# szy4017/DeepSense6G_TII

Measured on NVIDIA B200. Metric: train samples/sec (fwd+bwd), higher is better.
Workload: dtype bf16

## Files before the change

### deepsense6g_tii_b200/_capi.py

```python
import ctypes
import os
from ctypes import POINTER, c_char_p, c_double, c_float, c_int32, c_int64, c_void_p

import torch

_HERE = os.path.dirname(os.path.abspath(__file__))
LIB_PATH = os.environ.get("DSF_LIB") or os.path.join(_HERE, "libdsfuse.so")

DSF_F32, DSF_BF16 = 0, 1
DSF_NCHW, DSF_NHWC = 0, 1
EPI_BIAS, EPI_RELU, EPI_RESIDUAL, EPI_ACCUM = 1, 2, 4, 8

SYMBOLS = [
    "dsf_version", "dsf_last_error", "dsf_launch_count", "dsf_check_device", "dsf_set_pdl", "dsf_set_sm_margin", "dsf_dropout_inplace", "dsf_tokens_fwd", "dsf_tokens_bwd",
    "dsf_layernorm_fwd", "dsf_layernorm_bwd", "dsf_gemm_bf16_nt", "dsf_gemm_bf16_tn", "dsf_gemm_set_impl", "dsf_gemm_f32",
    "dsf_colsum", "dsf_relu_bwd", "dsf_relu_bwd_colsum", "dsf_pack_block_weights", "dsf_softmax_fwd", "dsf_softmax_bwd", "dsf_attn_fwd", "dsf_attn_bwd", "dsf_attn_bwd_parts", "dsf_attn_set_impl", "dsf_attn_drop_words",
    "dsf_upsample_add_fwd", "dsf_upsample_add_bwd", "dsf_cast_f32_bf16", "dsf_opt_tiles", "dsf_adamw_ema_pack", "dsf_opt_upload_table", "dsf_chain_fwd", "dsf_chain_bwd",
    "dsf_stem_pack", "dsf_tail_fwd", "dsf_tail_bwd",
]


class Geom(ctypes.Structure):
    _fields_ = [(n, c_int32) for n in ("B", "S", "V", "A_h", "A_w", "C", "H", "W", "feat_dtype", "layout")]

# ... 31 lines not shown
                "(there is no CPU / PyTorch fallback for the fusion stage)" % LIB_PATH)
        L = ctypes.CDLL(LIB_PATH)
        L.dsf_last_error.restype = c_char_p
        L.dsf_version.restype = c_int32
        L.dsf_launch_count.restype = c_int64
        P = c_void_p
        sig = {
            "dsf_check_device": [],
            "dsf_tokens_fwd": [POINTER(Geom), P, P, P, P, P, P, P],
            "dsf_tokens_bwd": [POINTER(Geom), P, P, P, P, P, P, P, P, P, P],
            "dsf_layernorm_fwd": [P, P, P, P, c_int32, P, P, c_int32, c_int32, c_float, P],
            "dsf_layernorm_bwd": [P, c_int32, P, P, P, P, P, P, P, P, P, P, POINTER(Dropout), c_int32, c_int32, P],
            "dsf_dropout_inplace": [P, c_int64, POINTER(Dropout), P],
            "dsf_relu_bwd_colsum": [P, P, P, c_int32, c_int32, P],
            "dsf_pack_block_weights": [P] * 9 + [c_int32, c_int32] + [P] * 10,
            "dsf_gemm_bf16_nt": [P, c_int32, P, c_int32, P, c_int32, c_int32, P, P, c_int32, c_int32, c_int32, c_int32, POINTER(Dropout), P, P],
            "dsf_gemm_bf16_tn": [P, c_int32, P, c_int32, P, c_int32, c_int32, c_int32, c_int32, P, P],
            "dsf_gemm_f32": [POINTER(GemmF32Desc), P, P, P, P, P, P],
            "dsf_colsum": [P, c_int32, c_int32, P, c_int32, c_int32, P],
            "dsf_relu_bwd": [P, P, c_int32, c_int64, P],
            "dsf_softmax_fwd": [P, c_int64, c_int32, P],
            "dsf_softmax_bwd": [P, P, c_int64, c_int32, P],
            "dsf_attn_fwd": [P, P, P, c_int32, c_int32, c_int32, c_int32, POINTER(Dropout), P, P],
            "dsf_attn_bwd": [P, P, P, P, P, P, c_int32, c_int32, c_int32, c_int32, POINTER(Dropout), P, P],
            "dsf_attn_bwd_parts": [P, P, P, P, P, P, c_int32, c_int32, c_int32, c_int32, POINTER(Dropout), P, c_int32, P],
            "dsf_attn_set_impl": [c_int32],
            "dsf_set_pdl": [c_int32],
            "dsf_set_sm_margin": [c_int32],
            "dsf_gemm_set_impl": [c_int32],
            "dsf_upsample_add_fwd": [POINTER(Geom), P, P, P, P, P, P, P, P],
            "dsf_upsample_add_bwd": [POINTER(Geom), P, P, P, P, P, P],
# ... 83 lines not shown
def dropout_inplace(x, drop):
    _chk(lib().dsf_dropout_inplace(_p(x), x.numel(), _dp(drop), _stream()), "dsf_dropout_inplace")


def relu_bwd_colsum(dy, h, out):
    M, N = dy.shape
    _chk(lib().dsf_relu_bwd_colsum(_p(dy), _p(h), _p(out), M, N, _stream()), "dsf_relu_bwd_colsum")


def pack_block_weights(wq, wk, wv, wp, w1, w2, bq, bk, bv, outs):
    C, F = wq.shape[0], w1.shape[0]
    _chk(lib().dsf_pack_block_weights(_p(wq), _p(wk), _p(wv), _p(wp), _p(w1), _p(w2), _p(bq), _p(bk), _p(bv), C, F,
                                      *[_p(t) for t in outs], _stream()), "dsf_pack_block_weights")


def gemm_bf16_nt(A, B, C, bias=None, residual=None, relu=False, drop=None, relu_src=None):
    M, K = A.shape
    N = B.shape[0]
    flags = (EPI_BIAS if bias is not None else 0) | (EPI_RELU if relu else 0) | (EPI_RESIDUAL if residual is not None else 0)
    _chk(lib().dsf_gemm_bf16_nt(_p(A), A.stride(0), _p(B), B.stride(0), _p(C), C.stride(0), _dt(C), _p(bias), _p(residual),
                                M, N, K, flags, _dp(drop), _p(relu_src), _stream()), "dsf_gemm_bf16_nt")


def gemm_bf16_tn(A, B, C, colsum=None):
    M, Nout = A.shape
    Kout = B.shape[1]
    _chk(lib().dsf_gemm_bf16_tn(_p(A), A.stride(0), _p(B), B.stride(0), _p(C), C.stride(0), M, Nout, Kout, _p(colsum), _stream()),
         "dsf_gemm_bf16_tn")


def gemm_f32(desc, A, B, C, bias=None, residual=None):
    _chk(lib().dsf_gemm_f32(ctypes.byref(desc), _p(A), _p(B), _p(C), _p(bias), _p(residual), _stream()), "dsf_gemm_f32")


def colsum(X, out):
    M, N = X.shape
# ... 120 lines not shown
```

### deepsense6g_tii_b200/csrc/attn_api.cu

```cuda
#include <algorithm>
#include <atomic>

#include "tc_common.cuh"

namespace dsf {


__global__ void __launch_bounds__(256)
attn_delta_kernel(const __nv_bfloat16* __restrict__ y, const __nv_bfloat16* __restrict__ dy, float* __restrict__ delta, int B, int T,
                  int C, int nh) {
  pdl_trigger();
  pdl_wait();
  const int lane = threadIdx.x & 31;
  const int hs = C / nh, gl = hs / 8;
  const int nchunk = C / 8;
  for (int64_t row = (int64_t)blockIdx.x * 8 + (threadIdx.x >> 5); row < (int64_t)B * T; row += (int64_t)gridDim.x * 8) {
    const int b = (int)(row / T), t = (int)(row % T);
    for (int c0 = 0; c0 < nchunk; c0 += 32) {
      const int ch = c0 + lane;
      float acc = 0.f;
      if (ch < nchunk) {
        const uint4 a = __ldg(reinterpret_cast<const uint4*>(y + row * C + ch * 8));
        const uint4 d = __ldg(reinterpret_cast<const uint4*>(dy + row * C + ch * 8));
        const __nv_bfloat162* ap = reinterpret_cast<const __nv_bfloat162*>(&a);
        const __nv_bfloat162* dp = reinterpret_cast<const __nv_bfloat162*>(&d);
#pragma unroll
        for (int k = 0; k < 4; ++k) {
          const float2 af = __bfloat1622float2(ap[k]), df = __bfloat1622float2(dp[k]);
          acc += af.x * df.x + af.y * df.y;
        }
      }
      for (int o = gl >> 1; o > 0; o >>= 1) acc += __shfl_xor_sync(0xffffffffu, acc, o);
      if (ch < nchunk && (lane % gl) == 0) delta[((size_t)b * nh + (ch * 8) / hs) * T + t] = acc;
    }
  }
}

int attn_fwd_run(const void* qkv, void* y, float* lse, int B, int T, int C, int nh, const dsf_dropout* drop, uint32_t* bits, int force_nwg,
                 cudaStream_t st);
int attn_bwd_run(const void* qkv, const void* y, const void* dy, const float* lse, float* delta, void* dqkv, int B, int T, int C, int nh,
                 const dsf_dropout* drop, uint32_t* bits, int parts, cudaStream_t st);

int run_attn_delta(const void* y, const void* dy, float* delta, int B, int T, int C, int nh, cudaStream_t st) {
  launch_pdl(attn_delta_kernel, dim3(std::min(cdiv(B * T, 8), num_sms() * 8)), dim3(256), 0, st, (const __nv_bfloat16*)y, (const __nv_bfloat16*)dy,
             delta, B, T, C, nh);
// ... 70 lines not shown
```

### deepsense6g_tii_b200/csrc/common.cuh

```cuda
#pragma once
#include <cuda_bf16.h>
#include <cuda_runtime.h>
#include <stdint.h>
#include <stdio.h>

#include "../../include/dsfuse.h"

namespace dsf {

void set_error(const char* fmt, ...);
int check_launch(const char* what);

#define DSF_REQUIRE(cond, ...)              \
  do {                                      \
    if (!(cond)) {                          \
      ::dsf::set_error(__VA_ARGS__);        \
      return DSF_EINVAL;                    \
    }                                       \
  } while (0)

inline bool aligned16(const void* p) { return (reinterpret_cast<uintptr_t>(p) & 15u) == 0; }
inline int cdiv(int a, int b) { return (a + b - 1) / b; }
inline int64_t cdiv64(int64_t a, int64_t b) { return (a + b - 1) / b; }

// ... 118 lines not shown
  }
}
__device__ __forceinline__ void drop_scale4(const DropArgs& a, uint64_t e4, float (&m)[4]) {
  float m8[8];
  drop_scale8(a, e4 >> 1, m8);
  const int h = (int)(e4 & 1) * 4;
#pragma unroll
  for (int k = 0; k < 4; ++k) m[k] = m8[h + k];
}

__device__ __forceinline__ uint32_t pack_bf16x2(float lo, float hi) {
  __nv_bfloat162 t = __floats2bfloat162_rn(lo, hi);
  return *reinterpret_cast<uint32_t*>(&t);
}

}
```

### deepsense6g_tii_b200/csrc/gemm_api.cu

```cuda
#include <algorithm>
#include <atomic>

#include "tc_common.cuh"

namespace dsf {

typedef CUresult (*PFN_encodeTiled)(CUtensorMap*, CUtensorMapDataType, cuuint32_t, void*, const cuuint64_t*, const cuuint64_t*,
                                    const cuuint32_t*, const cuuint32_t*, CUtensorMapInterleave, CUtensorMapSwizzle,
                                    CUtensorMapL2promotion, CUtensorMapFloatOOBfill);

static PFN_encodeTiled get_encode() {
  static PFN_encodeTiled fn = nullptr;
  if (!fn) {
    void* p = nullptr;
    cudaDriverEntryPointQueryResult q;
    if (cudaGetDriverEntryPoint("cuTensorMapEncodeTiled", &p, cudaEnableDefault, &q) == cudaSuccess && q == cudaDriverEntryPointSuccess)
      fn = (PFN_encodeTiled)p;
  }
  return fn;
}

int make_tmap_bf16(CUtensorMap* m, const void* base, int rows, int cols, int ld, int box_rows) {
  PFN_encodeTiled enc = get_encode();
  if (!enc) { set_error("cuTensorMapEncodeTiled entry point not available"); return DSF_ELAUNCH; }
// ... 14 lines not shown
  cuuint64_t gdim[2] = {(cuuint64_t)cols, (cuuint64_t)rows};
  cuuint64_t gstr[1] = {(cuuint64_t)ld * es};
  cuuint32_t box[2] = {(cuuint32_t)box_cols, (cuuint32_t)box_rows};
  cuuint32_t estr[2] = {1u, 1u};
  CUresult r = enc(m, dtype == DSF_F32 ? CU_TENSOR_MAP_DATA_TYPE_FLOAT32 : CU_TENSOR_MAP_DATA_TYPE_BFLOAT16, 2, const_cast<void*>(base), gdim,
                   gstr, box, estr, CU_TENSOR_MAP_INTERLEAVE_NONE, CU_TENSOR_MAP_SWIZZLE_128B, CU_TENSOR_MAP_L2_PROMOTION_L2_256B,
                   CU_TENSOR_MAP_FLOAT_OOB_FILL_NONE);
  if (r != CUDA_SUCCESS) { set_error("cuTensorMapEncodeTiled(2d) failed (%d) rows=%d cols=%d ld=%d box=%dx%d", (int)r, rows, cols, ld, box_cols, box_rows); return DSF_ELAUNCH; }
  return DSF_OK;
}

}

namespace dsf {
int gemm_nt_run(const void* A, int lda, const void* B, int ldb, void* C, int ldc, int c_dtype, const float* bias, const float* residual, int M,
                int N, int K, int flags, const dsf_dropout* drop, const void* relu_src, bool pairs, cudaStream_t st);
int gemm_tn_run(const void* A, int lda, const void* B, int ldb, float* C, int ldc, int M, int Nout, int Kout, float* colsum, cudaStream_t st);
static std::atomic<int> g_gemm_impl{0};
}

using namespace dsf;

extern "C" int dsf_gemm_set_impl(int32_t impl) {
  DSF_REQUIRE(impl == 0 || impl == 2, "gemm_set_impl: impl must be 0 (default: CTA pairs where the shape allows) or 2 (single-CTA tiles only)");
  g_gemm_impl.store(impl, std::memory_order_relaxed);
  return DSF_OK;
}

extern "C" int dsf_gemm_bf16_nt(const void* A, int32_t lda, const void* B, int32_t ldb, void* C, int32_t ldc, int32_t c_dtype,
                                const float* bias, const float* residual, int32_t M, int32_t N, int32_t K, int32_t epi_flags,
                                const dsf_dropout* drop, const void* relu_src, void* stream) {
  DSF_REQUIRE(A && B && C, "gemm_bf16_nt: NULL pointer");
  DSF_REQUIRE(M > 0 && N > 0 && K > 0, "gemm_bf16_nt: non-positive extent");
  DSF_REQUIRE(K % 64 == 0, "gemm_bf16_nt: K=%d must be a multiple of 64", K);
  DSF_REQUIRE(N % 64 == 0, "gemm_bf16_nt: N=%d must be a multiple of 64", N);
  DSF_REQUIRE(lda % 8 == 0 && ldb % 8 == 0 && ldc % 8 == 0 && lda >= K && ldb >= K && ldc >= N, "gemm_bf16_nt: bad leading dimensions");
  DSF_REQUIRE(aligned16(A) && aligned16(B) && aligned16(C) && aligned16(bias) && aligned16(residual), "gemm_bf16_nt: 16-byte alignment required");
  DSF_REQUIRE(c_dtype == DSF_F32 || c_dtype == DSF_BF16, "gemm_bf16_nt: bad c_dtype %d", c_dtype);
  DSF_REQUIRE(!(epi_flags & DSF_EPI_BIAS) || bias, "gemm_bf16_nt: bias flag without bias pointer");
  DSF_REQUIRE(!(epi_flags & DSF_EPI_RESIDUAL) || residual, "gemm_bf16_nt: residual flag without residual pointer");
  DSF_REQUIRE(!(epi_flags & DSF_EPI_ACCUM), "gemm_bf16_nt: ACCUM is not supported on the NT path");
  DSF_REQUIRE(!drop || (drop->p >= 0.f && drop->p < 1.f), "gemm_bf16_nt: dropout p must be in [0, 1)");
  DSF_REQUIRE(!relu_src || aligned16(relu_src), "gemm_bf16_nt: relu_src must be 16-byte aligned");
  return gemm_nt_run(A, lda, B, ldb, C, ldc, c_dtype, bias, residual, M, N, K, epi_flags, drop, relu_src,
                     g_gemm_impl.load(std::memory_order_relaxed) == 0, (cudaStream_t)stream);
}

extern "C" int dsf_gemm_bf16_tn(const void* A, int32_t lda, const void* B, int32_t ldb, float* C, int32_t ldc, int32_t M,
                                int32_t Nout, int32_t Kout, float* colsum_a, void* stream) {
  DSF_REQUIRE(A && B && C, "gemm_bf16_tn: NULL pointer");
  DSF_REQUIRE(M > 0 && Nout > 0 && Kout > 0, "gemm_bf16_tn: non-positive extent");
  DSF_REQUIRE(Nout % 64 == 0 && Kout % 64 == 0, "gemm_bf16_tn: output extents (%d, %d) must be multiples of 64", Nout, Kout);
  DSF_REQUIRE(lda % 8 == 0 && ldb % 8 == 0 && lda >= Nout && ldb >= Kout && ldc >= Kout, "gemm_bf16_tn: bad leading dimensions");
  DSF_REQUIRE(aligned16(A) && aligned16(B) && aligned16(C), "gemm_bf16_tn: 16-byte alignment required");
  return gemm_tn_run(A, lda, B, ldb, C, ldc, M, Nout, Kout, colsum_a, (cudaStream_t)stream);
}
```

### deepsense6g_tii_b200/csrc/gemm_tc2.cu

```cuda
#include <algorithm>
#include <cstdlib>

#include "tc_common.cuh"

namespace dsf {

using namespace tc;

int make_tmap_bf16(CUtensorMap* m, const void* base, int rows, int cols, int ld, int box_rows);
int make_tmap_2d(CUtensorMap* m, const void* base, int dtype, int rows, int cols, int ld, int box_cols, int box_rows);

constexpr int G2_BM = 128, G2_BK = 64, G2_THREADS = 320;

struct EpiArgs2 {
  void* C;
  int ldc;
  int c_dtype;
  const float* bias;
  const float* residual;
  int flags;
  int N;
  const __nv_bfloat16* relu_src;
  int ablate;
  DropArgs drop;
};

__device__ __forceinline__ void epi_store32(const EpiArgs2& e, int row, int n, const uint32_t (&r)[32]) {
  float v[32];
#pragma unroll
  for (int j = 0; j < 32; ++j) v[j] = __uint_as_float(r[j]);
  if (e.flags & DSF_EPI_BIAS) {
#pragma unroll
    for (int j = 0; j < 32; j += 4) {
      const float4 b = __ldg(reinterpret_cast<const float4*>(e.bias + n + j));
      v[j] += b.x; v[j + 1] += b.y; v[j + 2] += b.z; v[j + 3] += b.w;
    }
  }
  if (e.flags & DSF_EPI_RELU) {
#pragma unroll
// ... 53 lines not shown
#pragma unroll
    for (int j = 0; j < 32; j += 8) {
      float m[8];
      drop_scale8(e.drop, e8 + (j >> 3), m);
#pragma unroll
      for (int k = 0; k < 8; ++k) v[j + k] *= m[k];
    }
  }
  if ((e.flags & DSF_EPI_RESIDUAL) && row_ok) {
    const float4* rp = reinterpret_cast<const float4*>(e.residual + (size_t)row * e.ldc + n);
#pragma unroll
    for (int j = 0; j < 8; ++j) {
      const float4 t = rp[j];
      v[4 * j] += t.x; v[4 * j + 1] += t.y; v[4 * j + 2] += t.z; v[4 * j + 3] += t.w;
    }
  }
}

template <int BN, int STAGES, bool STAGED = true>
struct G2Smem {
  static constexpr int A_BYTES = G2_BM * G2_BK * 2;
  static constexpr int B_BYTES = BN * G2_BK * 2;
  static constexpr int STAGE_BYTES = A_BYTES + B_BYTES;
  static constexpr int STAGING_OFF = STAGES * STAGE_BYTES;
  static constexpr int STAGING_BYTES = STAGED ? 8 * 2 * 4096 : 0;
  static constexpr int BAR_OFF = STAGING_OFF + STAGING_BYTES;
  static constexpr int DYN = BAR_OFF + (2 * STAGES + 4) * 8 + 16 + 1024;
  static constexpr uint32_t TMEM_COLS = 2 * BN < 32 ? 32 : 2 * BN;
  static_assert(DYN <= 232448, "shared memory budget");
};
// ... 63 lines not shown
          if (elect_one()) {
#pragma unroll
            for (int k = 0; k < G2_BK / 16; ++k) tc_mma_bf16(acc, da + (uint32_t)(k * 2), db + (uint32_t)(k * 2), idesc, k == 0 ? first : 1u);
            tc_commit(bar_empty + s * 8);
          }
          __syncwarp();
        }
        if (elect_one()) tc_commit(acc_full + ab * 8);
        __syncwarp();
      }
    }
  } else {
    const int q = warp & 3;
    const int ch = (warp - 2) >> 2;
    epi.drop = resolve_drop(epi.drop);
    constexpr int NSPLIT = BN >= 128 ? 2 : 1;
    constexpr int HALF = BN / NSPLIT;
    int i = 0, nbox = 0;
    for (int tile = blockIdx.x; tile < total; tile += gridDim.x, ++i) {
      const int ab = i & 1;
      const int m0 = (tile % m_tiles) * G2_BM, n0 = (tile / m_tiles) * BN;
      mbar_wait(acc_full + ab * 8, (i >> 1) & 1);
      tc_fence_after();
      if (ch >= NSPLIT || m0 + q * 32 >= M || (epi.ablate & 1)) {
        tc_fence_before();
        __syncwarp();
        if (lane == 0) mbar_arrive(acc_empty + ab * 8);
        continue;
      }
      const int row = m0 + q * 32 + lane;
      const uint32_t tacc = tmem_base + ab * BN + ((uint32_t)(q * 32) << 16) + ch * HALF;
      const uint32_t stg = base + L::STAGING_OFF + (warp - 2) * 8192;
      const int CW = epi.c_dtype == DSF_F32 ? 32 : 64;
#pragma unroll 1
      for (int c = 0; c < HALF; c += CW, ++nbox) {
        const uint32_t sbuf = stg + (nbox & 1) * 4096;
        if (lane == 0) bulk_wait_read<1>();
        __syncwarp();
        const int ncol = n0 + ch * HALF + c;
        uint32_t w[32];
        if (epi.c_dtype == DSF_F32) {
          uint32_t r[32];
          tmem_ld32(tacc + c, r);
          tmem_wait_ld();
          float v[32];
          epi_math32(epi, row, ncol, r, v, row < M);
#pragma unroll
          for (int j = 0; j < 32; ++j) w[j] = __float_as_uint(v[j]);
        } else {
#pragma unroll
          for (int hh = 0; hh < 2; ++hh) {
            uint32_t r[32];
            tmem_ld32(tacc + c + hh * 32, r);
            tmem_wait_ld();
            float v[32];
            epi_math32(epi, row, ncol + hh * 32, r, v, row < M);
#pragma unroll
            for (int j = 0; j < 16; ++j) w[hh * 16 + j] = pack_bf16x2(v[2 * j], v[2 * j + 1]);
          }
        }
        if (!(epi.ablate & 8)) {
#pragma unroll
        for (int j = 0; j < 8; ++j) {
          const uint32_t dst = sbuf + lane * 128 + ((j ^ (lane & 7)) << 4);
          asm volatile("st.shared.v4.b32 [%0], {%1, %2, %3, %4};" ::"r"(dst), "r"(w[4 * j]), "r"(w[4 * j + 1]), "r"(w[4 * j + 2]), "r"(w[4 * j + 3])
                       : "memory");
        }
        fence_proxy_async();
        } else {
          uint32_t acc = 0;
#pragma unroll
          for (int j = 0; j < 32; ++j) acc ^= w[j];
          if (acc == 0x12345678u) asm volatile("st.shared.b32 [%0], %1;" ::"r"(sbuf), "r"(acc) : "memory");
        }
// ... 185 lines not shown
            for (int k = 0; k < G2_BK / 16; ++k) tc_mma_bf16_pair(acc, da + (uint32_t)(k * 2), db + (uint32_t)(k * 2), idesc, k == 0 ? first : 1u);
            tc_commit_pair(bar_empty + s * 8);
          }
          __syncwarp();
        }
        if (elect_one()) tc_commit_pair(acc_full + ab * 8);
        __syncwarp();
      }
    }
  } else {
    const int q = warp & 3;
    const int ch = (warp - 2) >> 2;
    epi.drop = resolve_drop(epi.drop);
    constexpr int HALF = BN / 2;
    const uint32_t acc_empty0 = mapa_u32(acc_empty, 0);
    int i = 0, nbox = 0;
    const uint32_t rbuf = base + L::RES_OFF + (warp - 2) * 4096, rbar = base + L::RBAR_OFF + (warp - 2) * 8;
    int nres = 0;
    bool r_inflight = false;
    auto chunks_of = [&](int uu, int& cm0, int& cn0, int& clo, int& chi) -> bool {
      int t2, a0, a1, p2, off2, w2;
      unit_of(uu, t2, a0, a1, p2);
      if (n_split > 1) nsub_of(uu, t2, off2, w2);
      else { off2 = 0; w2 = BN; }
      cm0 = (t2 % m_tiles) * 256 + (int)rank * G2_BM;
      cn0 = (t2 / m_tiles) * BN + off2;
      const int hu = w2 / 2;
      clo = hu >= 32 ? ch * hu : 0;
      chi = hu >= 32 ? clo + hu : (ch == 0 ? w2 : 0);
      return p2 == 0 && cm0 + q * 32 < M && !(epi.ablate & 1) && clo < chi;
// ... 6 lines not shown
      }
      r_inflight = true;
    };
    if (RTMA && pair < total) {
      int cm0, cn0, clo, chi;
      if (chunks_of(pair, cm0, cn0, clo, chi)) issue_res(cn0 + clo, cm0 + q * 32);
    }
    for (int u = pair; u < total; u += n_pairs, ++i) {
      int tile, kb0, kb1, part;
      unit_of(u, tile, kb0, kb1, part);
      int n_off, width;
      if (n_split > 1) nsub_of(u, tile, n_off, width);
      else { n_off = 0; width = BN; }
      const int ab = i & 1;
      const int m0 = (tile % m_tiles) * 256 + (int)rank * G2_BM, n0 = (tile / m_tiles) * BN + n_off;
      mbar_wait(acc_full + ab * 8, (i >> 1) & 1);
      tc_fence_after();
      if (part != 0) {
        const int row = m0 + q * 32 + lane;
        const uint32_t tacc = tmem_base + ab * BN + ((uint32_t)(q * 32) << 16) + ch * HALF;
        EpiArgs2 e2 = epi;
        if (part == 2) e2.flags &= ~(DSF_EPI_BIAS | DSF_EPI_RESIDUAL);
        if (m0 + q * 32 < M) {
#pragma unroll 1
          for (int c = 0; c < HALF; c += 32) {
            uint32_t r[32];
            tmem_ld32(tacc + c, r);
            tmem_wait_ld();
            float v[32];
            const int ncol = n0 + ch * HALF + c;
            epi_math32(e2, row, ncol, r, v, row < M);
            if (row < M) {
              float* cp = reinterpret_cast<float*>(epi.C) + (size_t)row * epi.ldc + ncol;
#pragma unroll
              for (int j = 0; j < 32; j += 4) red_add_v4(cp + j, v[j], v[j + 1], v[j + 2], v[j + 3]);
            }
          }
        }
      } else
      if (m0 + q * 32 < M && !(epi.ablate & 1)) {
        const int row = m0 + q * 32 + lane;
        const uint32_t tacc = tmem_base + ab * BN + ((uint32_t)(q * 32) << 16);
        const uint32_t stg = base + L::STAGING_OFF + (warp - 2) * 8192;
        const int CW = epi.c_dtype == DSF_F32 ? 32 : 64;
        const int half_u = width / 2;
        const int c_lo = half_u >= CW ? ch * half_u : 0;
        const int c_hi = half_u >= CW ? c_lo + half_u : (ch == 0 ? width : 0);
#pragma unroll 1
        for (int c = c_lo; c < c_hi; c += CW, ++nbox) {
          const uint32_t sbuf = stg + (nbox & 1) * 4096;
          if (lane == 0) bulk_wait_read<1>();
          __syncwarp();
          const int ncol = n0 + c;
          uint32_t w[32];
          if (RTMA) {
            if (!r_inflight) issue_res(ncol, m0 + q * 32);
            mbar_wait(rbar, nres & 1);
            ++nres;
            float rr[32];
#pragma unroll
            for (int j = 0; j < 8; ++j) {
              const uint32_t src = rbuf + lane * 128 + ((j ^ (lane & 7)) << 4);
// ... 13 lines not shown
            float v[32];
            EpiArgs2 e2 = epi;
            e2.flags &= ~DSF_EPI_RESIDUAL;
            epi_math32(e2, row, ncol, r, v, row < M);
#pragma unroll
            for (int j = 0; j < 32; ++j) w[j] = __float_as_uint(v[j] + rr[j]);
          } else if (epi.c_dtype == DSF_F32) {
            uint32_t r[32];
            tmem_ld32(tacc + c, r);
            tmem_wait_ld();
            float v[32];
            epi_math32(epi, row, ncol, r, v, row < M);
#pragma unroll
            for (int j = 0; j < 32; ++j) w[j] = __float_as_uint(v[j]);
          } else {
#pragma unroll
            for (int hh = 0; hh < 2; ++hh) {
              uint32_t r[32];
              tmem_ld32(tacc + c + hh * 32, r);
              tmem_wait_ld();
              float v[32];
              epi_math32(epi, row, ncol + hh * 32, r, v, row < M);
#pragma unroll
              for (int j = 0; j < 16; ++j) w[hh * 16 + j] = pack_bf16x2(v[2 * j], v[2 * j + 1]);
            }
          }
#pragma unroll
          for (int j = 0; j < 8; ++j) {
            const uint32_t dst = sbuf + lane * 128 + ((j ^ (lane & 7)) << 4);
            asm volatile("st.shared.v4.b32 [%0], {%1, %2, %3, %4};" ::"r"(dst), "r"(w[4 * j]), "r"(w[4 * j + 1]), "r"(w[4 * j + 2]), "r"(w[4 * j + 3])
                         : "memory");
          }
          fence_proxy_async();
          __syncwarp();
          if (lane == 0) {
            tma_store_2d(&tmC, sbuf, ncol, m0 + q * 32);
            bulk_commit();
          }
        }
      }
      tc_fence_before();
      __syncwarp();
      if (lane == 0) mbar_arrive_cluster(acc_empty0 + ab * 8);
    }
    if (lane == 0) bulk_wait<0>();
  }
  tc_fence_before();
  cluster_sync_all();
  if (warp == 1) tmem_dealloc_pair(tmem_base, L::TMEM_COLS);
}



template <int BN, int STAGES>
struct TnSmem : G2Smem<BN, STAGES, false> {
// ... 150 lines not shown
  const int tiles = cdiv(Nout, G2_BM) * cdiv(Kout, BN);
  int splits = std::max(1, std::min(cdiv(M, 2 * G2_BK), num_sms() / std::max(1, tiles)));
  int m_chunk = cdiv(cdiv(M, splits), G2_BK) * G2_BK;
  splits = cdiv(M, m_chunk);
  dim3 grid(cdiv(Kout, BN), cdiv(Nout, G2_BM), splits);
  launch_pdl(gemm_tn2_kernel<BN, STAGES>, grid, dim3(G2_THREADS), L::DYN, st, tmA, tmB, C, ldc, M, Nout, Kout, m_chunk, colsum);
  return check_launch("gemm_tn2");
}

static const bool g_nt_tail_nsplit = getenv("DSF_GEMM_TAIL_NSPLIT") ? atoi(getenv("DSF_GEMM_TAIL_NSPLIT")) != 0 : true;

static const bool g_nt_res_tma = getenv("DSF_GEMM_RES_TMA") ? atoi(getenv("DSF_GEMM_RES_TMA")) != 0 : true;

template <int BN, int STAGES, bool RTMA = false>
static int launch_nt3(const CUtensorMap& tmA, const CUtensorMap& tmB, const CUtensorMap& tmC, const EpiArgs2& epi, int M, int N, int K,
                      cudaStream_t st, const void* Bptr = nullptr, int ldb = 0) {
  using L = G3Smem<BN, STAGES, RTMA>;
  static bool configured_on[64] = {};
  bool& configured = per_device_flag(configured_on);
  if (!configured) {
    if (cudaFuncSetAttribute(gemm_nt3_kernel<BN, STAGES, RTMA>, cudaFuncAttributeMaxDynamicSharedMemorySize, L::DYN) != cudaSuccess)
      return check_launch("gemm_nt3/attr");
    configured = true;
  }
  CUtensorMap tmR = tmC;
  if (RTMA) {
    if (int e = make_tmap_2d(&tmR, epi.residual, DSF_F32, M, N, epi.ldc, 32, 32)) return e;
  }
  const int m_tiles = cdiv(M, 256), n_tiles = N / BN;
  const int tiles = m_tiles * n_tiles;
  const int pairs = std::min(tiles, num_sms() / 2);
  int tail_start = tiles;
  const int tail_split = 1;
  const int rem = tiles % pairs;
  int n_split = 1;
  CUtensorMap tmBt = tmB;
  if (g_nt_tail_nsplit && tail_split == 1 && BN == 256 && Bptr != nullptr && rem > 0 && tiles > pairs) {
    for (int ns = 4; ns >= 2; ns >>= 1) {
      if (rem * ns <= pairs) { n_split = ns; break; }
    }
    if (n_split > 1) {
      tail_start = tiles - rem;
      if (int e = make_tmap_bf16(&tmBt, Bptr, N, K, ldb, BN / n_split / 2)) return e;
    }
  }
  launch_pdl(gemm_nt3_kernel<BN, STAGES, RTMA>, dim3(2 * pairs), dim3(G2_THREADS), L::DYN, st, tmA, tmB, tmC, tmBt, tmR, epi, M, N, K, m_tiles,
             n_tiles, tail_start, tail_split, n_split);
  return check_launch("gemm_nt3");
}

static int pick_bn_nt(int M, int N) {
  const int sms = num_sms();
  const int m_tiles = cdiv(M, G2_BM);
  int best = 64;
  double best_cost = 1e30;
  const int cands[3] = {256, 128, 64};
  const double tile_eff[3] = {1.0, 0.85, 0.6};
  for (int i = 0; i < 3; ++i) {
    const int bn = cands[i];
    if (N % bn) continue;
    const int tiles = m_tiles * (N / bn);
    const double cost = (double)cdiv(tiles, sms) * bn / tile_eff[i];
    if (cost < best_cost) { best_cost = cost; best = bn; }
  }
  return best;
}

int gemm_nt_run(const void* A, int lda, const void* B, int ldb, void* C, int ldc, int c_dtype, const float* bias, const float* residual, int M,
                int N, int K, int flags, const dsf_dropout* drop, const void* relu_src, bool pairs, cudaStream_t st) {
  static const int ablate = [] {
    const int v = getenv("DSF_GEMM_ABLATE") ? atoi(getenv("DSF_GEMM_ABLATE")) : 0;
    if (v) fprintf(stderr, "dsfuse: DSF_GEMM_ABLATE=%d is set: tensor-core GEMM results are INVALID (timing diagnostics only)\n", v);
    return v;
  }();
  CUtensorMap tmA, tmB;
  if (pairs && N % 128 == 0 && M > 128) {
    const int BN3 = (N % 256 == 0) ? 256 : 128;
    if (int e = make_tmap_bf16(&tmA, A, M, K, lda, G2_BM)) return e;
    if (int e = make_tmap_bf16(&tmB, B, N, K, ldb, BN3 / 2)) return e;
    CUtensorMap tmC3;
    if (int e = make_tmap_2d(&tmC3, C, c_dtype, M, N, ldc, c_dtype == DSF_F32 ? 32 : 64, 32)) return e;
    EpiArgs2 epi3{C, ldc, c_dtype, bias, residual, flags, N, reinterpret_cast<const __nv_bfloat16*>(relu_src), ablate, make_drop(drop)};
    if (BN3 == 256 && g_nt_res_tma && c_dtype == DSF_F32 && (flags & DSF_EPI_RESIDUAL) && residual != nullptr && !ablate)
      return launch_nt3<256, 4, true>(tmA, tmB, tmC3, epi3, M, N, K, st, B, ldb);
    if (BN3 == 256) return launch_nt3<256, 5>(tmA, tmB, tmC3, epi3, M, N, K, st, B, ldb);
    if (g_nt_res_tma && c_dtype == DSF_F32 && (flags & DSF_EPI_RESIDUAL) && residual != nullptr && !ablate)
      return launch_nt3<128, 5, true>(tmA, tmB, tmC3, epi3, M, N, K, st);
    return launch_nt3<128, 6>(tmA, tmB, tmC3, epi3, M, N, K, st);
  }
  const int BN = pick_bn_nt(M, N);
  if (int e = make_tmap_bf16(&tmA, A, M, K, lda, G2_BM)) return e;
  if (int e = make_tmap_bf16(&tmB, B, N, K, ldb, BN)) return e;
  CUtensorMap tmC;
  if (int e = make_tmap_2d(&tmC, C, c_dtype, M, N, ldc, c_dtype == DSF_F32 ? 32 : 64, 32)) return e;
  EpiArgs2 epi{C, ldc, c_dtype, bias, residual, flags, N, reinterpret_cast<const __nv_bfloat16*>(relu_src), ablate, make_drop(drop)};
  if (BN == 256) return launch_nt2<256, 3>(tmA, tmB, tmC, epi, M, N, K, st);
  if (BN == 128) return launch_nt2<128, 4>(tmA, tmB, tmC, epi, M, N, K, st);
  return launch_nt2<64, 5>(tmA, tmB, tmC, epi, M, N, K, st);
}

int gemm_tn_run(const void* A, int lda, const void* B, int ldb, float* C, int ldc, int M, int Nout, int Kout, float* colsum, cudaStream_t st) {
  const int BN = (Kout % 256 == 0) ? 256 : ((Kout % 128 == 0) ? 128 : 64);
  CUtensorMap tmA, tmB;
  if (int e = make_tmap_bf16(&tmA, A, M, Nout, lda, G2_BK)) return e;
  if (int e = make_tmap_bf16(&tmB, B, M, Kout, ldb, G2_BK)) return e;
  if (BN == 256) return launch_tn2<256, 4>(tmA, tmB, C, ldc, M, Nout, Kout, colsum, st);
  if (BN == 128) return launch_tn2<128, 6>(tmA, tmB, C, ldc, M, Nout, Kout, colsum, st);
  return launch_tn2<64, 8>(tmA, tmB, C, ldc, M, Nout, Kout, colsum, st);
}

// ... 2 lines not shown
```

### deepsense6g_tii_b200/functional.py

```python
import math
import os

import torch
from torch.autograd.function import once_differentiable

from . import _capi as K
from ._capi import EPI_ACCUM, EPI_BIAS, EPI_RELU, EPI_RESIDUAL, GemmF32Desc

PER_BLOCK = ("ln1.weight", "ln1.bias", "ln2.weight", "ln2.bias",
             "attn.key.weight", "attn.key.bias", "attn.query.weight", "attn.query.bias",
             "attn.value.weight", "attn.value.bias", "attn.proj.weight", "attn.proj.bias",
             "mlp.0.weight", "mlp.0.bias", "mlp.2.weight", "mlp.2.bias")


def param_names(n_layer):
    names = ["pos_emb"]
    for i in range(n_layer):
        names += ["blocks.%d.%s" % (i, n) for n in PER_BLOCK]
    return names + ["ln_f.weight", "ln_f.bias"]


def _f32_linear_desc(M, N, Kd, flags, trans=None):
    return GemmF32Desc(M, N, Kd, 1, 1, 0, 0, Kd, 1, 0, 0, Kd, 1, 0, 0, N, 1, 1.0, flags)

# ... 358 lines not shown
            dwqkv, dwp, dw1, dw2, dbqkv, dbp, db1, db2, dg1, dbt1, dg2, dbt2 = block_views(i)
            dwqkv, dwp, dw1, dw2 = dwqkv.view(3 * C, C), dwp.view(C, C), dw1.view(F, C), dw2.view(C, F)
            fork(lambda: K.gemm_bf16_tn(dxa, st.a, dw2))
            da = torch.empty(M, F, device=dev, dtype=bf)
            K.gemm_bf16_nt(dxa, st.w2_t, da, relu_src=st.a)

            fork(lambda: K.gemm_bf16_tn(da, st.h2, dw1, colsum=db1))
            dh2 = torch.empty(M, C, device=dev, dtype=dh_dt)
            K.gemm_bf16_nt(da, st.w1_t, dh2)
            dx_mid = torch.empty(M, C, device=dev, dtype=f32)
            dxm = torch.empty(M, C, device=dev, dtype=bf)
            K.layernorm_bwd(dh2, st.x_mid, ln2w, st.mean2, st.rstd2, dx, dx_mid, dg2, dbt2, dx_bf16=dxm, dx_colsum=dbp,
                            byprod_drop=self._drop("proj", i))
            fork(lambda: K.gemm_bf16_tn(dxm, st.y, dwp))
            dy = torch.empty(M, C, device=dev, dtype=bf)
            K.gemm_bf16_nt(dxm, st.wp_t, dy)
            dqkv = torch.empty(M, 3 * C, device=dev, dtype=bf)
            delta = torch.empty(self.B, self.nh, self.T, device=dev, dtype=f32)
            if side is None:
                K.attn_bwd(st.qkv, st.y, dy, st.lse, delta, dqkv, self.B, self.T, C, self.nh, self._drop("attn", i), st.drop_bits)
            else:
                adrop = self._drop("attn", i)
                K.attn_bwd(st.qkv, st.y, dy, st.lse, delta, dqkv, self.B, self.T, C, self.nh, adrop, st.drop_bits, parts=1)
                fork(lambda: K.attn_bwd(st.qkv, st.y, dy, st.lse, delta, dqkv, self.B, self.T, C, self.nh, adrop, st.drop_bits, parts=4), side_q)
                K.attn_bwd(st.qkv, st.y, dy, st.lse, delta, dqkv, self.B, self.T, C, self.nh, adrop, st.drop_bits, parts=2)
                join(side_q)

            fork(lambda: K.gemm_bf16_tn(dqkv, st.h1, dwqkv, colsum=dbqkv))
            dh1 = torch.empty(M, C, device=dev, dtype=dh_dt)
            K.gemm_bf16_nt(dqkv, st.wqkv_t, dh1)
            join_pending()
            if side is not None:
                ev_blk = torch.cuda.Event()
                ev_blk.record(side)
                pending = (ev_blk, i, (st, da, dxm, dqkv))
            dx = torch.empty(M, C, device=dev, dtype=f32)
            prev = block_views(i - 1) if i > 0 else None
            K.layernorm_bwd(dh1, st.x_in, ln1w, st.mean1, st.rstd1, dx_mid, dx, dg1, dbt1,
# ... 387 lines not shown
```

### include/dsfuse.h

```cpp
#ifndef DSFUSE_H_
#define DSFUSE_H_

#include <stdint.h>

#ifdef __cplusplus
extern "C" {
#endif

#define DSF_VERSION 100

enum { DSF_F32 = 0, DSF_BF16 = 1 };
enum { DSF_NCHW = 0, DSF_NHWC = 1 };
enum {
  DSF_OK = 0,
  DSF_EINVAL = 1,
  DSF_ELAUNCH = 2,
  DSF_EARCH = 3,
  DSF_EUNSUPPORTED = 4
};

enum {
  DSF_EPI_BIAS = 1,
  DSF_EPI_RELU = 2,
  DSF_EPI_RESIDUAL = 4,
// ... 33 lines not shown

int dsf_tokens_bwd(const dsf_geom* g, const float* dx, const void* dres_img, const void* dres_lidar,
                   const void* dres_radar, void* dimg, void* dlidar, void* dradar, float* dgps,
                   float* dpos_emb, void* stream);

int dsf_layernorm_fwd(const float* x, const float* gamma, const float* beta, void* y, int32_t y_dtype,
                      float* mean, float* rstd, int32_t M, int32_t C, float eps, void* stream);
int dsf_layernorm_bwd(const void* dy, int32_t dy_dtype, const float* x, const float* gamma,
                      const float* mean, const float* rstd, const float* dx_add, float* dx_out,
                      float* dgamma, float* dbeta, void* dx_bf16, float* dx_colsum,
                      const dsf_dropout* byprod_drop, int32_t M, int32_t C, void* stream);

int dsf_gemm_bf16_nt(const void* A, int32_t lda, const void* B, int32_t ldb, void* C, int32_t ldc,
                     int32_t c_dtype, const float* bias, const float* residual, int32_t M, int32_t N,
                     int32_t K, int32_t epi_flags, const dsf_dropout* drop, const void* relu_src,
                     void* stream);
int dsf_gemm_bf16_tn(const void* A, int32_t lda, const void* B, int32_t ldb, float* C, int32_t ldc,
                     int32_t M, int32_t Nout, int32_t Kout, float* colsum_a, void* stream);
int dsf_gemm_set_impl(int32_t impl);

typedef struct {
  int32_t M, N, K;
  int32_t nb1, nb2;
  int64_t a_b1, a_b2, a_m, a_k;
  int64_t b_b1, b_b2, b_n, b_k;
  int64_t c_b1, c_b2, c_m, c_n;
  float alpha;
  int32_t epi_flags;
} dsf_gemm_f32_desc;
int dsf_gemm_f32(const dsf_gemm_f32_desc* d, const float* A, const float* B, float* C,
                 const float* bias, const float* residual, void* stream);
// ... 80 lines not shown
```

Baseline: 1321.

## Fuse attention-backward delta row-dot into the dy GEMM epilogue

The GEMM that produces dy = dxm·Wp^T now also computes the per-head row dot product of dy with y in its epilogue and writes delta directly. This removes the separate delta pass that re-read y and dy (attn_bwd parts 1/6 now skip it). The epilogue gains extra y loads and reductions, and the tile width choices are constrained so each tile covers whole head groups, which may lower GEMM efficiency.

```diff
diff --git a/deepsense6g_tii_b200/_capi.py b/deepsense6g_tii_b200/_capi.py
--- a/deepsense6g_tii_b200/_capi.py
+++ b/deepsense6g_tii_b200/_capi.py
@@ -69,7 +69,8 @@
             "dsf_dropout_inplace": [P, c_int64, POINTER(Dropout), P],
             "dsf_relu_bwd_colsum": [P, P, P, c_int32, c_int32, P],
             "dsf_pack_block_weights": [P] * 9 + [c_int32, c_int32] + [P] * 10,
-            "dsf_gemm_bf16_nt": [P, c_int32, P, c_int32, P, c_int32, c_int32, P, P, c_int32, c_int32, c_int32, c_int32, POINTER(Dropout), P, P],
+            "dsf_gemm_bf16_nt": [P, c_int32, P, c_int32, P, c_int32, c_int32, P, P, c_int32, c_int32, c_int32, c_int32, POINTER(Dropout), P,
+                                 P, P, c_int32, c_int32, P],
             "dsf_gemm_bf16_tn": [P, c_int32, P, c_int32, P, c_int32, c_int32, c_int32, c_int32, P, P],
             "dsf_gemm_f32": [POINTER(GemmF32Desc), P, P, P, P, P, P],
             "dsf_colsum": [P, c_int32, c_int32, P, c_int32, c_int32, P],
@@ -183,12 +184,20 @@
                                       *[_p(t) for t in outs], _stream()), "dsf_pack_block_weights")
 
 
-def gemm_bf16_nt(A, B, C, bias=None, residual=None, relu=False, drop=None, relu_src=None):
+def gemm_bf16_nt(A, B, C, bias=None, residual=None, relu=False, drop=None, relu_src=None, dot_src=None, dot_out=None):
     M, K = A.shape
     N = B.shape[0]
     flags = (EPI_BIAS if bias is not None else 0) | (EPI_RELU if relu else 0) | (EPI_RESIDUAL if residual is not None else 0)
+    dot_T = dot_nh = 0
+    if dot_out is not None:
+        _req(dot_out, torch.float32, "dot_out")
+        if (dot_out.dim() != 3 or dot_out.shape[0] * dot_out.shape[2] != M or dot_src is None or dot_src.dtype != torch.bfloat16
+                or dot_src.shape != C.shape or dot_src.stride() != C.stride()):
+            raise RuntimeError("gemm_bf16_nt: dot_out must be (B, nh, T) with B*T = M rows and dot_src bf16 with C's shape and strides")
+        dot_nh, dot_T = dot_out.shape[1], dot_out.shape[2]
     _chk(lib().dsf_gemm_bf16_nt(_p(A), A.stride(0), _p(B), B.stride(0), _p(C), C.stride(0), _dt(C), _p(bias), _p(residual),
-                                M, N, K, flags, _dp(drop), _p(relu_src), _stream()), "dsf_gemm_bf16_nt")
+                                M, N, K, flags, _dp(drop), _p(relu_src), _p(dot_src), _p(dot_out), dot_T, dot_nh, _stream()),
+         "dsf_gemm_bf16_nt")
 
 
 def gemm_bf16_tn(A, B, C, colsum=None):
diff --git a/deepsense6g_tii_b200/csrc/attn_api.cu b/deepsense6g_tii_b200/csrc/attn_api.cu
--- a/deepsense6g_tii_b200/csrc/attn_api.cu
+++ b/deepsense6g_tii_b200/csrc/attn_api.cu
@@ -22,13 +22,7 @@
       if (ch < nchunk) {
         const uint4 a = __ldg(reinterpret_cast<const uint4*>(y + row * C + ch * 8));
         const uint4 d = __ldg(reinterpret_cast<const uint4*>(dy + row * C + ch * 8));
-        const __nv_bfloat162* ap = reinterpret_cast<const __nv_bfloat162*>(&a);
-        const __nv_bfloat162* dp = reinterpret_cast<const __nv_bfloat162*>(&d);
-#pragma unroll
-        for (int k = 0; k < 4; ++k) {
-          const float2 af = __bfloat1622float2(ap[k]), df = __bfloat1622float2(dp[k]);
-          acc += af.x * df.x + af.y * df.y;
-        }
+        acc = dot8_bf16(a, d);
       }
       for (int o = gl >> 1; o > 0; o >>= 1) acc += __shfl_xor_sync(0xffffffffu, acc, o);
       if (ch < nchunk && (lane % gl) == 0) delta[((size_t)b * nh + (ch * 8) / hs) * T + t] = acc;
diff --git a/deepsense6g_tii_b200/csrc/common.cuh b/deepsense6g_tii_b200/csrc/common.cuh
--- a/deepsense6g_tii_b200/csrc/common.cuh
+++ b/deepsense6g_tii_b200/csrc/common.cuh
@@ -156,4 +156,16 @@
   return *reinterpret_cast<uint32_t*>(&t);
 }
 
+__device__ __forceinline__ float dot8_bf16(const uint4& a, const uint4& b) {
+  const uint32_t aw[4] = {a.x, a.y, a.z, a.w}, bw[4] = {b.x, b.y, b.z, b.w};
+  float acc = 0.f;
+#pragma unroll
+  for (int k = 0; k < 4; ++k) {
+    const float2 af = __bfloat1622float2(*reinterpret_cast<const __nv_bfloat162*>(&aw[k]));
+    const float2 bf = __bfloat1622float2(*reinterpret_cast<const __nv_bfloat162*>(&bw[k]));
+    acc = __fadd_rn(acc, __fmaf_rn(af.x, bf.x, __fmul_rn(af.y, bf.y)));
+  }
+  return acc;
 }
+
+}
diff --git a/deepsense6g_tii_b200/csrc/gemm_api.cu b/deepsense6g_tii_b200/csrc/gemm_api.cu
--- a/deepsense6g_tii_b200/csrc/gemm_api.cu
+++ b/deepsense6g_tii_b200/csrc/gemm_api.cu
@@ -52,7 +52,8 @@
 
 namespace dsf {
 int gemm_nt_run(const void* A, int lda, const void* B, int ldb, void* C, int ldc, int c_dtype, const float* bias, const float* residual, int M,
-                int N, int K, int flags, const dsf_dropout* drop, const void* relu_src, bool pairs, cudaStream_t st);
+                int N, int K, int flags, const dsf_dropout* drop, const void* relu_src, const void* dot_src, float* dot_out, int dot_T, int dot_nh,
+                bool pairs, cudaStream_t st);
 int gemm_tn_run(const void* A, int lda, const void* B, int ldb, float* C, int ldc, int M, int Nout, int Kout, float* colsum, cudaStream_t st);
 static std::atomic<int> g_gemm_impl{0};
 }
@@ -67,7 +68,8 @@
 
 extern "C" int dsf_gemm_bf16_nt(const void* A, int32_t lda, const void* B, int32_t ldb, void* C, int32_t ldc, int32_t c_dtype,
                                 const float* bias, const float* residual, int32_t M, int32_t N, int32_t K, int32_t epi_flags,
-                                const dsf_dropout* drop, const void* relu_src, void* stream) {
+                                const dsf_dropout* drop, const void* relu_src, const void* dot_src, float* dot_out, int32_t dot_T,
+                                int32_t dot_nh, void* stream) {
   DSF_REQUIRE(A && B && C, "gemm_bf16_nt: NULL pointer");
   DSF_REQUIRE(M > 0 && N > 0 && K > 0, "gemm_bf16_nt: non-positive extent");
   DSF_REQUIRE(K % 64 == 0, "gemm_bf16_nt: K=%d must be a multiple of 64", K);
@@ -80,7 +82,18 @@
   DSF_REQUIRE(!(epi_flags & DSF_EPI_ACCUM), "gemm_bf16_nt: ACCUM is not supported on the NT path");
   DSF_REQUIRE(!drop || (drop->p >= 0.f && drop->p < 1.f), "gemm_bf16_nt: dropout p must be in [0, 1)");
   DSF_REQUIRE(!relu_src || aligned16(relu_src), "gemm_bf16_nt: relu_src must be 16-byte aligned");
-  return gemm_nt_run(A, lda, B, ldb, C, ldc, c_dtype, bias, residual, M, N, K, epi_flags, drop, relu_src,
+  if (dot_out) {
+    DSF_REQUIRE(dot_src && aligned16(dot_src) && reinterpret_cast<uintptr_t>(dot_out) % 4 == 0,
+                "gemm_bf16_nt: the row-dot output needs a 16-byte aligned dot_src and a 4-byte aligned dot_out");
+    DSF_REQUIRE(c_dtype == DSF_BF16, "gemm_bf16_nt: the row-dot output needs a bf16 C");
+    DSF_REQUIRE(epi_flags == 0 && !(drop && drop->p > 0.f) && !relu_src,
+                "gemm_bf16_nt: the row-dot output does not combine with bias / ReLU / residual / dropout / relu_src");
+    DSF_REQUIRE(dot_nh > 0 && N % dot_nh == 0, "gemm_bf16_nt: row-dot groups: N=%d is not a multiple of nh=%d", N, dot_nh);
+    const int hs = N / dot_nh;
+    DSF_REQUIRE(hs == 16 || hs == 32 || hs == 64 || hs == 128, "gemm_bf16_nt: row-dot group width N/nh=%d not supported (16, 32, 64, 128)", hs);
+    DSF_REQUIRE(dot_T > 0 && M % dot_T == 0, "gemm_bf16_nt: row-dot: M=%d is not B*T for T=%d", M, dot_T);
+  }
+  return gemm_nt_run(A, lda, B, ldb, C, ldc, c_dtype, bias, residual, M, N, K, epi_flags, drop, relu_src, dot_src, dot_out, dot_T, dot_nh,
                      g_gemm_impl.load(std::memory_order_relaxed) == 0, (cudaStream_t)stream);
 }
 
diff --git a/deepsense6g_tii_b200/csrc/gemm_tc2.cu b/deepsense6g_tii_b200/csrc/gemm_tc2.cu
--- a/deepsense6g_tii_b200/csrc/gemm_tc2.cu
+++ b/deepsense6g_tii_b200/csrc/gemm_tc2.cu
@@ -23,6 +23,9 @@
   const __nv_bfloat16* relu_src;
   int ablate;
   DropArgs drop;
+  const __nv_bfloat16* dot_src;
+  float* dot_out;
+  int dot_hs, dot_T;
 };
 
 __device__ __forceinline__ void epi_store32(const EpiArgs2& e, int row, int n, const uint32_t (&r)[32]) {
@@ -106,6 +109,63 @@
       const float4 t = rp[j];
       v[4 * j] += t.x; v[4 * j + 1] += t.y; v[4 * j + 2] += t.z; v[4 * j + 3] += t.w;
     }
+  }
+}
+
+template <int N>
+__device__ __forceinline__ float butterfly_sum(const float* p) {
+  if constexpr (N == 1) {
+    return p[0];
+  } else {
+    float b[N / 2];
+#pragma unroll
+    for (int i = 0; i < N / 2; ++i) b[i] = p[i] + p[i + N / 2];
+    return butterfly_sum<N / 2>(b);
+  }
+}
+
+__device__ __forceinline__ void rowdot_store(const EpiArgs2& e, int row, int M, int n, float v) {
+  if (row >= M) return;
+  const int b = row / e.dot_T, t = row - b * e.dot_T;
+  e.dot_out[((size_t)b * (e.N / e.dot_hs) + n / e.dot_hs) * e.dot_T + t] = v;
+}
+
+__device__ __forceinline__ void rowdot_load64(const EpiArgs2& e, int row, int M, int n, uint4 (&s)[8]) {
+  if (row < M) {
+    const uint4* p = reinterpret_cast<const uint4*>(e.dot_src + (size_t)row * e.ldc + n);
+#pragma unroll
+    for (int j = 0; j < 8; ++j) s[j] = __ldg(p + j);
+  } else {
+#pragma unroll
+    for (int j = 0; j < 8; ++j) s[j] = make_uint4(0u, 0u, 0u, 0u);
+  }
+}
+
+__device__ __forceinline__ void rowdot_prefetch(const EpiArgs2& e, int row, int M, int n, int cols) {
+  if (row >= M) return;
+  const char* p = reinterpret_cast<const char*>(e.dot_src + (size_t)row * e.ldc + n);
+  for (int off = 0; off < cols * 2; off += 128) asm volatile("prefetch.global.L2 [%0];" ::"l"(p + off));
+}
+
+__device__ __forceinline__ void rowdot64(const EpiArgs2& e, int row, int M, int n, const uint32_t (&w)[32], const uint4 (&s)[8], float (&carry)[8]) {
+  float p[8];
+#pragma unroll
+  for (int j = 0; j < 8; ++j) p[j] = dot8_bf16(make_uint4(w[4 * j], w[4 * j + 1], w[4 * j + 2], w[4 * j + 3]), s[j]);
+  if (e.dot_hs == 16) {
+#pragma unroll
+    for (int k = 0; k < 4; ++k) rowdot_store(e, row, M, n + 16 * k, butterfly_sum<2>(p + 2 * k));
+  } else if (e.dot_hs == 32) {
+#pragma unroll
+    for (int k = 0; k < 2; ++k) rowdot_store(e, row, M, n + 32 * k, butterfly_sum<4>(p + 4 * k));
+  } else if (e.dot_hs == 64) {
+    rowdot_store(e, row, M, n, butterfly_sum<8>(p));
+  } else if ((n & 127) == 0) {
+#pragma unroll
+    for (int j = 0; j < 8; ++j) carry[j] = p[j];
+  } else {
+#pragma unroll
+    for (int j = 0; j < 8; ++j) p[j] = carry[j] + p[j];
+    rowdot_store(e, row, M, n - 64, butterfly_sum<8>(p));
   }
 }
 
@@ -199,12 +259,14 @@
     const int q = warp & 3;
     const int ch = (warp - 2) >> 2;
     epi.drop = resolve_drop(epi.drop);
-    constexpr int NSPLIT = BN >= 128 ? 2 : 1;
-    constexpr int HALF = BN / NSPLIT;
+    const bool rowdot = epi.dot_out != nullptr;
+    const int NSPLIT = BN >= 128 && (!rowdot || BN / 2 >= epi.dot_hs) ? 2 : 1;
+    const int HALF = BN / NSPLIT;
     int i = 0, nbox = 0;
     for (int tile = blockIdx.x; tile < total; tile += gridDim.x, ++i) {
       const int ab = i & 1;
       const int m0 = (tile % m_tiles) * G2_BM, n0 = (tile / m_tiles) * BN;
+      if (rowdot) rowdot_prefetch(epi, m0 + q * 32 + lane, M, n0 + ch * (BN / 2), BN / 2);
       mbar_wait(acc_full + ab * 8, (i >> 1) & 1);
       tc_fence_after();
       if (ch >= NSPLIT || m0 + q * 32 >= M || (epi.ablate & 1)) {
@@ -217,6 +279,7 @@
       const uint32_t tacc = tmem_base + ab * BN + ((uint32_t)(q * 32) << 16) + ch * HALF;
       const uint32_t stg = base + L::STAGING_OFF + (warp - 2) * 8192;
       const int CW = epi.c_dtype == DSF_F32 ? 32 : 64;
+      float rd_carry[8];
 #pragma unroll 1
       for (int c = 0; c < HALF; c += CW, ++nbox) {
         const uint32_t sbuf = stg + (nbox & 1) * 4096;
@@ -233,6 +296,8 @@
 #pragma unroll
           for (int j = 0; j < 32; ++j) w[j] = __float_as_uint(v[j]);
         } else {
+          uint4 ds[8];
+          if (rowdot) rowdot_load64(epi, row, M, ncol, ds);
 #pragma unroll
           for (int hh = 0; hh < 2; ++hh) {
             uint32_t r[32];
@@ -243,6 +308,7 @@
 #pragma unroll
             for (int j = 0; j < 16; ++j) w[hh * 16 + j] = pack_bf16x2(v[2 * j], v[2 * j + 1]);
           }
+          if (rowdot) rowdot64(epi, row, M, ncol, w, ds, rd_carry);
         }
         if (!(epi.ablate & 8)) {
 #pragma unroll
@@ -458,6 +524,7 @@
     epi.drop = resolve_drop(epi.drop);
     constexpr int HALF = BN / 2;
     const uint32_t acc_empty0 = mapa_u32(acc_empty, 0);
+    const bool rowdot = epi.dot_out != nullptr;
     int i = 0, nbox = 0;
     const uint32_t rbuf = base + L::RES_OFF + (warp - 2) * 4096, rbar = base + L::RBAR_OFF + (warp - 2) * 8;
     int nres = 0;
@@ -494,6 +561,7 @@
       else { n_off = 0; width = BN; }
       const int ab = i & 1;
       const int m0 = (tile % m_tiles) * 256 + (int)rank * G2_BM, n0 = (tile / m_tiles) * BN + n_off;
+      if (rowdot) rowdot_prefetch(epi, m0 + q * 32 + lane, M, n0 + ch * (width / 2), width / 2);
       mbar_wait(acc_full + ab * 8, (i >> 1) & 1);
       tc_fence_after();
       if (part != 0) {
@@ -524,8 +592,10 @@
         const uint32_t stg = base + L::STAGING_OFF + (warp - 2) * 8192;
         const int CW = epi.c_dtype == DSF_F32 ? 32 : 64;
         const int half_u = width / 2;
-        const int c_lo = half_u >= CW ? ch * half_u : 0;
-        const int c_hi = half_u >= CW ? c_lo + half_u : (ch == 0 ? width : 0);
+        const bool halves = half_u >= CW && (!rowdot || half_u >= epi.dot_hs);
+        const int c_lo = halves ? ch * half_u : 0;
+        const int c_hi = halves ? c_lo + half_u : (ch == 0 ? width : 0);
+        float rd_carry[8];
 #pragma unroll 1
         for (int c = c_lo; c < c_hi; c += CW, ++nbox) {
           const uint32_t sbuf = stg + (nbox & 1) * 4096;
@@ -569,6 +639,8 @@
 #pragma unroll
             for (int j = 0; j < 32; ++j) w[j] = __float_as_uint(v[j]);
           } else {
+            uint4 ds[8];
+            if (rowdot) rowdot_load64(epi, row, M, ncol, ds);
 #pragma unroll
             for (int hh = 0; hh < 2; ++hh) {
               uint32_t r[32];
@@ -579,6 +651,7 @@
 #pragma unroll
               for (int j = 0; j < 16; ++j) w[hh * 16 + j] = pack_bf16x2(v[2 * j], v[2 * j + 1]);
             }
+            if (rowdot) rowdot64(epi, row, M, ncol, w, ds, rd_carry);
           }
 #pragma unroll
           for (int j = 0; j < 8; ++j) {
@@ -593,7 +666,7 @@
             bulk_commit();
           }
         }
-      }
+        }
       tc_fence_before();
       __syncwarp();
       if (lane == 0) mbar_arrive_cluster(acc_empty0 + ab * 8);
@@ -774,7 +847,7 @@
 
 template <int BN, int STAGES, bool RTMA = false>
 static int launch_nt3(const CUtensorMap& tmA, const CUtensorMap& tmB, const CUtensorMap& tmC, const EpiArgs2& epi, int M, int N, int K,
-                      cudaStream_t st, const void* Bptr = nullptr, int ldb = 0) {
+                      cudaStream_t st, const void* Bptr = nullptr, int ldb = 0, int min_width = 0) {
   using L = G3Smem<BN, STAGES, RTMA>;
   static bool configured_on[64] = {};
   bool& configured = per_device_flag(configured_on);
@@ -797,7 +870,7 @@
   CUtensorMap tmBt = tmB;
   if (g_nt_tail_nsplit && tail_split == 1 && BN == 256 && Bptr != nullptr && rem > 0 && tiles > pairs) {
     for (int ns = 4; ns >= 2; ns >>= 1) {
-      if (rem * ns <= pairs) { n_split = ns; break; }
+      if (rem * ns <= pairs && BN / ns >= min_width) { n_split = ns; break; }
     }
     if (n_split > 1) {
       tail_start = tiles - rem;
@@ -809,7 +882,7 @@
   return check_launch("gemm_nt3");
 }
 
-static int pick_bn_nt(int M, int N) {
+static int pick_bn_nt(int M, int N, int min_bn) {
   const int sms = num_sms();
   const int m_tiles = cdiv(M, G2_BM);
   int best = 64;
@@ -818,7 +891,7 @@
   const double tile_eff[3] = {1.0, 0.85, 0.6};
   for (int i = 0; i < 3; ++i) {
     const int bn = cands[i];
-    if (N % bn) continue;
+    if (N % bn || bn < min_bn) continue;
     const int tiles = m_tiles * (N / bn);
     const double cost = (double)cdiv(tiles, sms) * bn / tile_eff[i];
     if (cost < best_cost) { best_cost = cost; best = bn; }
@@ -827,33 +900,38 @@
 }
 
 int gemm_nt_run(const void* A, int lda, const void* B, int ldb, void* C, int ldc, int c_dtype, const float* bias, const float* residual, int M,
-                int N, int K, int flags, const dsf_dropout* drop, const void* relu_src, bool pairs, cudaStream_t st) {
+                int N, int K, int flags, const dsf_dropout* drop, const void* relu_src, const void* dot_src, float* dot_out, int dot_T, int dot_nh,
+                bool pairs, cudaStream_t st) {
   static const int ablate = [] {
     const int v = getenv("DSF_GEMM_ABLATE") ? atoi(getenv("DSF_GEMM_ABLATE")) : 0;
     if (v) fprintf(stderr, "dsfuse: DSF_GEMM_ABLATE=%d is set: tensor-core GEMM results are INVALID (timing diagnostics only)\n", v);
     return v;
   }();
   CUtensorMap tmA, tmB;
+  const int dot_hs = dot_out ? N / dot_nh : 0;
+  const __nv_bfloat16* dsrc = reinterpret_cast<const __nv_bfloat16*>(dot_src);
   if (pairs && N % 128 == 0 && M > 128) {
     const int BN3 = (N % 256 == 0) ? 256 : 128;
     if (int e = make_tmap_bf16(&tmA, A, M, K, lda, G2_BM)) return e;
     if (int e = make_tmap_bf16(&tmB, B, N, K, ldb, BN3 / 2)) return e;
     CUtensorMap tmC3;
     if (int e = make_tmap_2d(&tmC3, C, c_dtype, M, N, ldc, c_dtype == DSF_F32 ? 32 : 64, 32)) return e;
-    EpiArgs2 epi3{C, ldc, c_dtype, bias, residual, flags, N, reinterpret_cast<const __nv_bfloat16*>(relu_src), ablate, make_drop(drop)};
+    EpiArgs2 epi3{C, ldc, c_dtype, bias, residual, flags, N, reinterpret_cast<const __nv_bfloat16*>(relu_src), ablate, make_drop(drop),
+                  dsrc, dot_out, dot_hs, dot_T};
     if (BN3 == 256 && g_nt_res_tma && c_dtype == DSF_F32 && (flags & DSF_EPI_RESIDUAL) && residual != nullptr && !ablate)
       return launch_nt3<256, 4, true>(tmA, tmB, tmC3, epi3, M, N, K, st, B, ldb);
-    if (BN3 == 256) return launch_nt3<256, 5>(tmA, tmB, tmC3, epi3, M, N, K, st, B, ldb);
+    if (BN3 == 256) return launch_nt3<256, 5>(tmA, tmB, tmC3, epi3, M, N, K, st, B, ldb, dot_hs);
     if (g_nt_res_tma && c_dtype == DSF_F32 && (flags & DSF_EPI_RESIDUAL) && residual != nullptr && !ablate)
       return launch_nt3<128, 5, true>(tmA, tmB, tmC3, epi3, M, N, K, st);
     return launch_nt3<128, 6>(tmA, tmB, tmC3, epi3, M, N, K, st);
   }
-  const int BN = pick_bn_nt(M, N);
+  const int BN = pick_bn_nt(M, N, dot_hs);
   if (int e = make_tmap_bf16(&tmA, A, M, K, lda, G2_BM)) return e;
   if (int e = make_tmap_bf16(&tmB, B, N, K, ldb, BN)) return e;
   CUtensorMap tmC;
   if (int e = make_tmap_2d(&tmC, C, c_dtype, M, N, ldc, c_dtype == DSF_F32 ? 32 : 64, 32)) return e;
-  EpiArgs2 epi{C, ldc, c_dtype, bias, residual, flags, N, reinterpret_cast<const __nv_bfloat16*>(relu_src), ablate, make_drop(drop)};
+  EpiArgs2 epi{C, ldc, c_dtype, bias, residual, flags, N, reinterpret_cast<const __nv_bfloat16*>(relu_src), ablate, make_drop(drop),
+               dsrc, dot_out, dot_hs, dot_T};
   if (BN == 256) return launch_nt2<256, 3>(tmA, tmB, tmC, epi, M, N, K, st);
   if (BN == 128) return launch_nt2<128, 4>(tmA, tmB, tmC, epi, M, N, K, st);
   return launch_nt2<64, 5>(tmA, tmB, tmC, epi, M, N, K, st);
diff --git a/deepsense6g_tii_b200/functional.py b/deepsense6g_tii_b200/functional.py
--- a/deepsense6g_tii_b200/functional.py
+++ b/deepsense6g_tii_b200/functional.py
@@ -396,14 +396,13 @@
                             byprod_drop=self._drop("proj", i))
             fork(lambda: K.gemm_bf16_tn(dxm, st.y, dwp))
             dy = torch.empty(M, C, device=dev, dtype=bf)
-            K.gemm_bf16_nt(dxm, st.wp_t, dy)
+            delta = torch.empty(self.B, self.nh, self.T, device=dev, dtype=f32)
+            K.gemm_bf16_nt(dxm, st.wp_t, dy, dot_src=st.y, dot_out=delta)
             dqkv = torch.empty(M, 3 * C, device=dev, dtype=bf)
-            delta = torch.empty(self.B, self.nh, self.T, device=dev, dtype=f32)
+            adrop = self._drop("attn", i)
             if side is None:
-                K.attn_bwd(st.qkv, st.y, dy, st.lse, delta, dqkv, self.B, self.T, C, self.nh, self._drop("attn", i), st.drop_bits)
+                K.attn_bwd(st.qkv, st.y, dy, st.lse, delta, dqkv, self.B, self.T, C, self.nh, adrop, st.drop_bits, parts=6)
             else:
-                adrop = self._drop("attn", i)
-                K.attn_bwd(st.qkv, st.y, dy, st.lse, delta, dqkv, self.B, self.T, C, self.nh, adrop, st.drop_bits, parts=1)
                 fork(lambda: K.attn_bwd(st.qkv, st.y, dy, st.lse, delta, dqkv, self.B, self.T, C, self.nh, adrop, st.drop_bits, parts=4), side_q)
                 K.attn_bwd(st.qkv, st.y, dy, st.lse, delta, dqkv, self.B, self.T, C, self.nh, adrop, st.drop_bits, parts=2)
                 join(side_q)
diff --git a/include/dsfuse.h b/include/dsfuse.h
--- a/include/dsfuse.h
+++ b/include/dsfuse.h
@@ -71,7 +71,7 @@
 int dsf_gemm_bf16_nt(const void* A, int32_t lda, const void* B, int32_t ldb, void* C, int32_t ldc,
                      int32_t c_dtype, const float* bias, const float* residual, int32_t M, int32_t N,
                      int32_t K, int32_t epi_flags, const dsf_dropout* drop, const void* relu_src,
-                     void* stream);
+                     const void* dot_src, float* dot_out, int32_t dot_T, int32_t dot_nh, void* stream);
 int dsf_gemm_bf16_tn(const void* A, int32_t lda, const void* B, int32_t ldb, float* C, int32_t ldc,
                      int32_t M, int32_t Nout, int32_t Kout, float* colsum_a, void* stream);
 int dsf_gemm_set_impl(int32_t impl);
```

After: 1322, median of 6. No clear change (+0.1%).
